# mlcolab/Pathfinder.jl

Measured on AMD Instinct MI355X. Metric: ELBO draws/sec (multipathfinder hot path: fit + ELBO + pool + PSIS + resample), higher is better.
Workload: dtype f64

## Files before the change

pathfinder.jl_amd/csrc/elbo_qf_kernel.hip:

```cpp
#include <type_traits>
#include <stdio.h>
#include <stdlib.h>
#include "pfmi_common.h"
#include "elbo_args.h"
#ifndef QF_PROF
#define QF_PROF 0
#endif

#ifndef QF_WAVES
#define QF_WAVES 8
#endif
#define QF_THREADS (QF_WAVES * 64)
#ifndef QF_NG
#define QF_NG 2
#endif
#ifndef QF_ABLATE
#define QF_ABLATE 0
#endif
#ifndef QF_PHILOX_HOIST
#define QF_PHILOX_HOIST 1
#endif
#ifndef QF_PSEUDO_FLIGHT
#define QF_PSEUDO_FLIGHT 1
#endif
#ifndef QF_CS_LDS
#define QF_CS_LDS 1
#endif
#ifndef QF_NG2_MAXKC
#define QF_NG2_MAXKC 20
#endif
#ifndef QF_PRIO_FAIR
#define QF_PRIO_FAIR 8
#endif
#ifndef QF_PRIO_YOUNG
#define QF_PRIO_YOUNG 0
#endif
#ifndef QF_SETPRIO
#define QF_SETPRIO 0
#endif
#define QF_MIN_FRONT 1024
static_assert(QF_MIN_FRONT >= 2 * PF_ICDF_BFE_FRONT, "the look-up's front guard");
template <int KC> struct qf_chb { static constexpr int v = (KC > 20) ? 8 : 16; };

#pragma clang fp contract(off)

typedef double qf_d4 __attribute__((ext_vector_type(4)));
__device__ __forceinline__ qf_d4 qf_mfma16(double a, double b, qf_d4 c) { return __builtin_amdgcn_mfma_f64_16x16x4f64(a, b, c, 0, 0, 0); }
__device__ __forceinline__ double qf_mfma4(double a, double b, double c) { return __builtin_amdgcn_mfma_f64_4x4x4f64(a, b, c, 0, 0, 0); }

__host__ __device__ constexpr int qf_nconst(int KC, int RPAD) { return 4 + KC + KC * KC + RPAD + RPAD * KC + KC; }

__host__ __device__ constexpr int qf_head_lds(int KC, int NG) { return (NG == 2 && KC < 16) ? 256 : 0; }

template <int TGT>
__device__ __forceinline__ void qf_row_ac(const ElboArgs &A, const double *mu, int i, double &a, double &c) {
    if (TGT == 1) { a = A.t_a[i]; c = mu[i] - A.t_mean[i]; }
    else if (TGT == 2) { a = (i >= 1) ? 1.0 : 0.0; c = mu[i]; }
    else { a = 0.0; c = 0.0; }
}

template <int KC>
__device__ __forceinline__ int qf_vh_pos(int lrow, int col) {
    const int bl = lrow >> 4, rr = lrow & 15, q = rr >> 2, r = rr & 3, T = col >> 2, i = col & 3;
    return (((bl * 4 + r) * (KC / 4) + T) << 4) + q * 4 + i;
}

struct QfKernArgs { ElboArgs A; int ch_blocks, nchunks, groups_per_wg, ngroups, n_whole, n_tail, ndep; double *cshare; unsigned *cflag; unsigned epoch; int cs_off; };
__host__ __device__ constexpr bool qf_cs_lds(int KC, int TGT, int NG) { return QF_CS_LDS != 0 && TGT != 0 && !(NG == 2 && KC >= 16); }
__device__ __forceinline__ int qf_arg_cs_off() {
    const char *ka = (const char *)__builtin_amdgcn_kernarg_segment_ptr();
    asm volatile("" : "+s"(ka));
    return *reinterpret_cast<const int *>(ka + offsetof(QfKernArgs, cs_off));
}
#ifndef QF_SHARE_SPINS
#define QF_SHARE_SPINS 2000000
#endif
template <int KC, int TGT, int RPAD, int NG>
__global__ __launch_bounds__(QF_THREADS) void pf_elbo_qf_kernel(ElboArgs A, int ch_blocks, int nchunks, int groups_per_wg, int ngroups, int n_whole,
                                                                  int n_tail, int ndep, double *, unsigned *, unsigned, int) {
    extern __shared__ __attribute__((aligned(16))) double lds[];
#if QF_PROF
    const long long qf_t0 = wall_clock64();
    long long qf_tb = 0, qf_te = 0, qf_tp = 0, qf_last = 0;
#endif
    constexpr int NT = KC / 4, TR = RPAD / 4, NC = qf_nconst(KC, RPAD);
    constexpr int QF_CHB = qf_chb<KC>::v;
    constexpr bool FOLD = !(NG == 2 && KC >= 16);
    constexpr bool PHX = QF_PHILOX_HOIST != 0;
    constexpr int PRE = (QF_CHB * 16 * KC + QF_THREADS - 1) / QF_THREADS;
    const int tid = threadIdx.x, wv = tid >> 6, lane = tid & 63, q = lane >> 4, c = lane & 15, l3 = lane & 3;
    const int d = A.d, nblk = (d + 15) >> 4;
    int slot = blockIdx.y, role = 0;
    int g_begin = blockIdx.x * groups_per_wg, g_cap = groups_per_wg;
    if (n_tail > 0 && slot >= n_whole) {
        constexpr int SL = QF_WAVES * NG, NPG_ = (TGT != 0) ? (KC + 1 + 15) / 16 : 0;
        int tail_f;
        if (slot < n_whole + n_tail) { role = 1; tail_f = slot - n_whole; g_begin = 0; g_cap = SL - NPG_; }
        else {
            const int t = slot - n_whole - n_tail;
            role = 2; tail_f = t / ndep;
            g_begin = (SL - NPG_) + (t - tail_f * ndep) * SL; g_cap = SL;
        }
        slot = n_whole + tail_f;
    }
    const int p = A.points[slot];
    const size_t blkidx = A.by_point ? (size_t)p : (size_t)slot;
    double *out_lp = A.logp + blkidx * A.log_stride, *out_lq = A.logq + blkidx * A.log_stride;
    constexpr int NPG = (TGT != 0) ? (KC + 1 + 15) / 16 : 0;
    const int npg = (role == 2) ? 0 : NPG;
    const int g_end = (g_begin + g_cap < ngroups) ? g_begin + g_cap : ngroups;
    const int nlb = (npg + (g_end - g_begin) + QF_WAVES * NG - 1) / (QF_WAVES * NG);
    if (A.status[p] != PFMI_FIT_OK) {
        for (int64_t n = (int64_t)g_begin * 16 + tid; n < (int64_t)g_end * 16 && n < A.N; n += QF_THREADS) {
            out_lp[n] = NAN; out_lq[n] = NAN;
        }
        return;
    }
    const int vh_sz = ch_blocks * 16 * KC, rs_sz = ch_blocks * 48;
    const int buf_stride = (nchunks > 1) ? vh_sz + rs_sz : 0;
    const int stage_sz = (nchunks > 1 ? 2 : 1) * (vh_sz + rs_sz);
    const int fix_off = stage_sz > QF_MIN_FRONT ? stage_sz : QF_MIN_FRONT;
    double *t_s = lds + fix_off;
    double *cn_s = t_s + KC * KC;
    double *g_s = cn_s + NC;
    double *h_s = g_s + RPAD * RPAD;
    double2 *icdf = reinterpret_cast<double2 *>(h_s + qf_head_lds(KC, NG) + ((KC * KC + NC + RPAD * RPAD) & 1));

    const double *Vh = A.vh + (size_t)p * d * KC, *mu = A.mu + (size_t)p * d, *sqa = A.sqrt_alpha + (size_t)p * d;
    auto stage_direct = [&](int ck, int buf) {
        const int row0 = ck * ch_blocks * 16;
        double *vs = lds + buf * buf_stride, *rs = vs + vh_sz;
        const int npair = ch_blocks * 8 * KC;
        const int lim = (d - row0) * KC;
        const double2 *src = reinterpret_cast<const double2 *>(Vh + (size_t)row0 * KC);
        constexpr int U = 6;
        for (int j0 = tid; j0 < npair; j0 += QF_THREADS * U) {
            double2 v[U];
#pragma unroll
            for (int u = 0; u < U; ++u) {
                const int j = j0 + u * QF_THREADS, jc = (2 * j + 1 < lim) ? j : (lim >> 1) - 1;
                v[u] = src[jc];
            }
#pragma unroll
            for (int u = 0; u < U; ++u) {
                const int j = j0 + u * QF_THREADS, idx = 2 * j;
                if (j < npair) {
                    const int lrow = idx / KC, col = idx - lrow * KC;
                    const double2 val = (idx < lim) ? v[u] : make_double2(0.0, 0.0);
                    *reinterpret_cast<double2 *>(vs + qf_vh_pos<KC>(lrow, col)) = val;
                }
            }
        }
        int cs_o = 0;
        if constexpr (qf_cs_lds(KC, TGT, NG)) { if (npg > 0) cs_o = qf_arg_cs_off(); }
        for (int l0 = tid; l0 < ch_blocks * 16; l0 += QF_THREADS * 2) {
            double a[2], cc[2], s[2];
#pragma unroll
            for (int u = 0; u < 2; ++u) {
                const int lrow = l0 + u * QF_THREADS, row = row0 + lrow, rc = row < d ? row : d - 1;
                qf_row_ac<TGT>(A, mu, rc, a[u], cc[u]);
                s[u] = sqa[rc];
            }
#pragma unroll
            for (int u = 0; u < 2; ++u) {
                const int lrow = l0 + u * QF_THREADS, row = row0 + lrow;
                if (lrow < ch_blocks * 16) {
                    const bool in = row < d;
                    double *o = rs + (lrow >> 4) * 48 + (lrow & 15);
                    o[0] = in ? a[u] * s[u] * s[u] : 0.0; o[16] = in ? 2.0 * a[u] * cc[u] * s[u] : 0.0; o[32] = in ? s[u] : 0.0;
                    if constexpr (qf_cs_lds(KC, TGT, NG)) { if (cs_o) lds[cs_o + lrow] = in ? cc[u] / s[u] : 0.0; }
                }
            }
        }
    };
    {
        const double *T = A.tmat + (size_t)p * KC * KC;
        for (int i = tid; i < KC * KC; i += QF_THREADS) t_s[i] = T[i];
        for (int i = tid; i < NC; i += QF_THREADS) cn_s[i] = 0.0;
        if (RPAD > 0) for (int i = tid; i < RPAD * RPAD; i += QF_THREADS) g_s[i] = A.t_g[i];
        pf_icdf_load(icdf);
        stage_direct(0, 0);
    }
    const int rho = 4 * (c & 3) + (c >> 2);
    constexpr bool HLDS = qf_head_lds(KC, NG) > 0;
    constexpr bool HREG = !(NG == 2 && KC >= 16) && !HLDS;
    const double *Vc = A.vchol + (size_t)p * KC * KC;
    auto head_op = [&](const int which, const int r) -> double {
        const int b = 4 * q + r;
        if (which == 0) { double v = (rho == b) ? 1.0 : 0.0; if (rho < KC && b < KC) v = Vc[b * KC + rho]; return v; }
        const int i1 = 16 + rho, b1 = 16 + b;
        if (which == 1) return (i1 < KC) ? Vc[b * KC + i1] : 0.0;
        double v1 = (i1 == b1) ? 1.0 : 0.0;
        if (i1 < KC && b1 < KC) v1 = Vc[b1 * KC + i1];
        return v1;
    };
    double a_h00[HREG ? 4 : 1], a_h10[HREG ? 4 : 1], a_h11[HREG ? 4 : 1];
    if (HREG) {
#pragma unroll
        for (int r = 0; r < 4; ++r) {
            a_h00[HREG ? r : 0] = head_op(0, r);
            a_h10[HREG ? r : 0] = (KC > 16) ? head_op(1, r) : 0.0;
            a_h11[HREG ? r : 0] = (KC > 16) ? head_op(2, r) : 0.0;
        }
    }
    if (HLDS && wv == 0) {
#pragma unroll
        for (int r = 0; r < 4; ++r) h_s[r * 64 + lane] = head_op(0, r);
    }
    auto hop = [&](const int which, const int r) -> double {
        if (HLDS) return h_s[r * 64 + lane];
        if (HREG) return which == 0 ? a_h00[HREG ? r : 0] : (which == 1 ? a_h10[HREG ? r : 0] : a_h11[HREG ? r : 0]);
        return head_op(which, r);
    };
    const uint64_t seed = A.seeds[slot];
    const uint32_t k0 = (uint32_t)seed, k1 = (uint32_t)(seed >> 32);
    const double logdet = A.logdet[p];
    __syncthreads();
#if QF_PROF
    qf_tp = wall_clock64() - qf_t0; qf_last = wall_clock64();
#endif
#if QF_PRIO_YOUNG
    if (wv >= 4) __builtin_amdgcn_s_setprio(1);
#endif
    if (TGT == 2) {
        if (tid == 0) { cn_s[1] = mu[0]; cn_s[2] = sqa[0]; }
        if (tid < KC) cn_s[4 + KC + KC * KC + RPAD + RPAD * KC + tid] = Vh[tid];
    }

    int cur = 0;
    for (int lb = 0; lb < nlb; ++lb) {
        bool pseudo[NG], active[NG];
        int sl[NG];
        int grp[NG];
        pf_philox_inv pinv[NG];
        auto draw_of = [&](const int g) -> uint32_t { return (uint32_t)(A.n0 + ((int64_t)grp[g] * 16 + c)); };
        double accw[NG][NT], acc3[NG][NT], acc4[NG][TR > 0 ? TR : 1];
        double usq[NG], q12[NG], z00[NG], u0[NG][4];
        bool any_active = false, any_pseudo = false, any_real = false;
#pragma unroll
        for (int g = 0; g < NG; ++g) {
            sl[g] = (lb * QF_WAVES + wv) * NG + g;
            pseudo[g] = sl[g] < npg;
            grp[g] = g_begin + sl[g] - npg;
            active[g] = pseudo[g] || grp[g] < g_end;
            if (PHX) {
                pinv[g] = pf_philox_draw_invariants(draw_of(g), k0, k1);
                if constexpr (NG == 2 && KC >= 16) asm volatile("" : "+v"(pinv[g].C), "+v"(pinv[g].D), "+v"(pinv[g].E), "+v"(pinv[g].F));
            }
            any_active |= active[g]; any_pseudo |= pseudo[g]; any_real |= active[g] && !pseudo[g];
#pragma unroll
            for (int T = 0; T < NT; ++T) { accw[g][T] = 0.0; acc3[g][T] = 0.0; }
#pragma unroll
            for (int T = 0; T < (TR > 0 ? TR : 1); ++T) acc4[g][T] = 0.0;
            usq[g] = 0.0; q12[g] = 0.0; z00[g] = 0.0;
#pragma unroll
            for (int r = 0; r < 4; ++r) u0[g][r] = 0.0;
        }
        struct Pend { uint32_t x[4]; double dp[4]; double2 c01[4], c23[4]; };
        const uint32_t icdf_adj = pf_icdf_adj_bfe<PF_ICDF_NB_LDS>(icdf);
        auto gen_issue = [&](const int g, const int blk, const uint64_t t, Pend &P) {
            auto words = [&](uint32_t (&x)[4]) {
                if (PHX) pf_philox4x32_hoisted<PF_NORMAL_ROUNDS>(pinv[g], t, k0, k1, x);
                else pf_philox_normals(draw_of(g), (uint32_t)(blk * 4 + q), 0u, 0u, k0, k1, x);
            };
#if QF_ABLATE == 1
#pragma unroll
            for (int r = 0; r < 4; ++r) { P.x[r] = 0x40000000u | (draw_of(g) + blk); P.dp[r] = 1e-3 * (blk + r); P.c01[r] = make_double2(0.1, 0.2); P.c23[r] = make_double2(0.3, 0.4); }
#elif QF_ABLATE == 2
            words(P.x);
#pragma unroll
            for (int r = 0; r < 4; ++r) { P.dp[r] = (double)P.x[r] * 0x1p-32; P.c01[r] = make_double2(0.1, 0.2); P.c23[r] = make_double2(0.3, 0.4); }
#else
            words(P.x);
#pragma unroll
            for (int r = 0; r < 4; ++r) pf_icdf_issue_bfe<PF_ICDF_NB_LDS>(P.x[r], icdf_adj, P.dp[r], P.c01[r], P.c23[r]);
#endif
        };
        for (int ck = 0; ck < nchunks; ++ck) {
            double pre[PRE], pr_s = 0.0, pr_a = 0.0, pr_c = 0.0;
            const int nck = (ck + 1 < nchunks) ? ck + 1 : 0;
            const bool do_pre = (nchunks > 1) && (ck + 1 < nchunks || lb + 1 < nlb);
            if (do_pre) {
                const int row0 = nck * QF_CHB * 16;
                int tid_p = tid;
                asm volatile("" : "+v"(tid_p));
#pragma unroll
                for (int e = 0; e < PRE; ++e) {
                    const int idx = tid_p + e * QF_THREADS;
                    const int lrow = idx / KC, row = row0 + lrow;
                    pre[e] = (idx < QF_CHB * 16 * KC && row < d) ? Vh[(size_t)row0 * KC + idx] : 0.0;
                }
                if (tid_p < QF_CHB * 16) {
                    const int row = row0 + tid_p;
                    if (row < d) { qf_row_ac<TGT>(A, mu, row, pr_a, pr_c); pr_s = sqa[row]; }
                }
            }
            if (any_active) {
                const double *vs = lds + cur * buf_stride, *rs = vs + vh_sz;
                const int blk0 = ck * ch_blocks;
                const int nb = (nblk - blk0 < ch_blocks) ? nblk - blk0 : ch_blocks;
                struct Ops { double av[4][NT]; double wd[4][TR > 0 ? TR : 1]; double rs[12]; };
                auto load_ops = [&](const int bl, Ops &o) {
                    const double *rp = rs + bl * 48 + 4 * q;
                    const double *ap = vs + ((bl * 4) * NT << 4) + q * 4 + l3;
#pragma unroll
                    for (int r = 0; r < 4; ++r) {
#pragma unroll
                        for (int T = 0; T < NT; ++T) o.av[r][T] = ap[(r * NT + T) << 4];
                        o.rs[r] = rp[r]; o.rs[4 + r] = rp[16 + r]; o.rs[8 + r] = rp[32 + r];
                    }
                    if (TGT == 1 && RPAD > 0) {
                        const double *wp = A.t_wd16 + ((size_t)(blk0 + bl) * 16 + 4 * q) * 16 + l3;
#pragma unroll
                        for (int r = 0; r < 4; ++r)
#pragma unroll
                            for (int T = 0; T < TR; ++T) o.wd[r][T] = wp[r * 16 + 4 * T];
                    }
                };
                auto contract = [&](const int g, const double (&z)[4], const Ops &o, const bool with_w) {
#if QF_SETPRIO
                    __builtin_amdgcn_s_setprio(QF_SETPRIO);
#endif
                    double bp[4], bs[4];
#pragma unroll
                    for (int r = 0; r < 4; ++r) {
                        bp[r] = 0.0; bs[r] = 0.0;
                        if (TGT != 0) bp[r] = (with_w && FOLD) ? fma(o.rs[r], z[r], o.rs[4 + r]) : o.rs[r] * z[r];
                        if (TGT == 1 && RPAD > 0) bs[r] = o.rs[8 + r] * z[r];
                    }
                    __builtin_amdgcn_sched_barrier(0);
#pragma unroll
                    for (int r = 0; r < 4; ++r) {
                        if (TGT != 0) q12[g] = fma((with_w && FOLD) ? bp[r] : bp[r] + o.rs[4 + r], z[r], q12[g]);
#pragma unroll
                        for (int T = 0; T < NT; ++T) {
                            if (with_w) accw[g][T] = qf_mfma4(o.av[r][T], z[r], accw[g][T]);
                            if (TGT != 0) acc3[g][T] = qf_mfma4(o.av[r][T], bp[r], acc3[g][T]);
                        }
                        if (TGT == 1 && RPAD > 0) {
#pragma unroll
                            for (int T = 0; T < TR; ++T) acc4[g][T] = qf_mfma4(o.wd[r][T], bs[r], acc4[g][T]);
                        }
                    }
#if QF_SETPRIO
                    __builtin_amdgcn_s_setprio(0);
#endif
                };
                auto normals = [&](const int g, const int blk, double (&z)[4]) {
                    uint32_t x[4];
                    pf_philox_normals(draw_of(g), (uint32_t)(blk * 4 + q), 0u, 0u, k0, k1, x);
                    pf_icdf4(x, draw_of(g), (uint32_t)(blk * 4 + q), 0u, k0, k1, icdf, z);
                    if (blk == nblk - 1) {
#pragma unroll
                        for (int r = 0; r < 4; ++r) z[r] = (blk * 16 + 4 * q + r < d) ? z[r] : 0.0;
                    }
#pragma unroll
                    for (int r = 0; r < 4; ++r) usq[g] = fma(z[r], z[r], usq[g]);
                    if (blk == 0) {
                        qf_d4 h = {0.0, 0.0, 0.0, 0.0};
#pragma unroll
                        for (int r = 0; r < 4; ++r) { u0[g][r] = z[r]; h = qf_mfma16(hop(0, r), z[r], h); }
#pragma unroll
                        for (int r = 0; r < 4; ++r) z[r] = h[r];
                        z00[g] = z[0];
                    } else if (KC > 16 && blk == 1) {
                        qf_d4 h = {0.0, 0.0, 0.0, 0.0};
#pragma unroll
                        for (int r = 0; r < 4; ++r) h = qf_mfma16(hop(1, r), u0[g][r], h);
#pragma unroll
                        for (int r = 0; r < 4; ++r) h = qf_mfma16(hop(2, r), z[r], h);
#pragma unroll
                        for (int r = 0; r < 4; ++r) z[r] = h[r];
                    }
                };
                auto finish = [&](const int g, const int blk, const Pend &P, double (&z)[4], auto special_tag) {
                    constexpr bool SPECIAL = decltype(special_tag)::value;
#pragma unroll
                    for (int r = 0; r < 4; ++r) z[r] = pf_icdf_finish(P.x[r], P.dp[r], P.c01[r], P.c23[r]);
                    if (__builtin_expect(__any(pf_icdf_miss4(P.x)), 0))
                        pf_icdf4_fix(P.x, draw_of(g), (uint32_t)(blk * 4 + q), 0u, k0, k1, z);
                    if (SPECIAL) {
                        if (blk == nblk - 1) {
#pragma unroll
                            for (int r = 0; r < 4; ++r) z[r] = (blk * 16 + 4 * q + r < d) ? z[r] : 0.0;
                        }
#pragma unroll
                        for (int r = 0; r < 4; ++r) usq[g] = fma(z[r], z[r], usq[g]);
                        if (blk == 0) {
                            qf_d4 h = {0.0, 0.0, 0.0, 0.0};
#pragma unroll
                            for (int r = 0; r < 4; ++r) { u0[g][r] = z[r]; h = qf_mfma16(hop(0, r), z[r], h); }
#pragma unroll
                            for (int r = 0; r < 4; ++r) z[r] = h[r];
                            z00[g] = z[0];
                        } else if (KC > 16 && blk == 1) {
                            qf_d4 h = {0.0, 0.0, 0.0, 0.0};
#pragma unroll
                            for (int r = 0; r < 4; ++r) h = qf_mfma16(hop(1, r), u0[g][r], h);
#pragma unroll
                            for (int r = 0; r < 4; ++r) h = qf_mfma16(hop(2, r), z[r], h);
#pragma unroll
                            for (int r = 0; r < 4; ++r) z[r] = h[r];
                        }
                    } else {
#pragma unroll
                        for (int r = 0; r < 4; ++r) usq[g] = fma(z[r], z[r], usq[g]);
                    }
                };
                auto pseudo_cols = [&](const int g, const int blk, const int bl, const int cs_o, double (&z)[4]) {
                    const int j = 16 * sl[g] + c;
                    if (qf_cs_lds(KC, TGT, NG) && cs_o != 0) {
                        const double *cs = lds + cs_o + bl * 16 + 4 * q;
#pragma unroll
                        for (int r = 0; r < 4; ++r) {
                            double v = 0.0;
                            if (j < KC) v = vs[qf_vh_pos<KC>(bl * 16 + 4 * q + r, j)];
                            else if (j == KC) v = cs[r];
                            z[r] = v;
                        }
                    } else if constexpr (QF_PSEUDO_FLIGHT != 0 && TGT == 1) {
                        double pm[4], ptm[4], ps[4];
#pragma unroll
                        for (int r = 0; r < 4; ++r) {
                            const int row = blk * 16 + 4 * q + r, rc = row < d ? row : d - 1;
                            pm[r] = mu[rc]; ptm[r] = A.t_mean[rc]; ps[r] = sqa[rc];
                        }
                        asm volatile("" ::: "memory");
                        __builtin_amdgcn_sched_barrier(0);
#pragma unroll
                        for (int r = 0; r < 4; ++r) {
                            const int row = blk * 16 + 4 * q + r;
                            double v = 0.0;
                            if (j < KC) v = vs[qf_vh_pos<KC>(bl * 16 + 4 * q + r, j)];
                            else if (j == KC && row < d) v = (pm[r] - ptm[r]) / ps[r];
                            z[r] = v;
                        }
                    } else {
#pragma unroll
                        for (int r = 0; r < 4; ++r) {
                            const int row = blk * 16 + 4 * q + r;
                            double v = 0.0;
                            if (j < KC) v = vs[qf_vh_pos<KC>(bl * 16 + 4 * q + r, j)];
                            else if (j == KC && row < d) {
                                double aa, cc;
                                qf_row_ac<TGT>(A, mu, row, aa, cc);
                                v = cc / sqa[row];
                            }
                            z[r] = v;
                        }
                    }
                };
                if (any_pseudo) {
                    int cs_o = 0;
                    if constexpr (qf_cs_lds(KC, TGT, NG)) cs_o = qf_arg_cs_off();
                    for (int bl = 0; bl < nb; ++bl) {
                        Ops oa;
                        load_ops(bl, oa);
#pragma unroll
                        for (int g = 0; g < NG; ++g) {
                            if (!active[g]) continue;
                            double z[4];
                            if (pseudo[g]) { pseudo_cols(g, blk0 + bl, bl, cs_o, z); contract(g, z, oa, false); }
                            else { normals(g, blk0 + bl, z); contract(g, z, oa, true); }
                        }
                    }
                } else {
                    auto block_body_seq = [&](const int bl, auto special_tag) {
                        const int blk = blk0 + bl;
                        double z[NG][4];
                        const uint64_t t = pf_philox_block_product((uint32_t)(blk * 4 + q), k0);
#pragma unroll
                        for (int g = 0; g < NG; ++g) {
                            Pend pp;
                            gen_issue(g, blk, t, pp);
                            finish(g, blk, pp, z[g], special_tag);
                        }
                        const double *rp = rs + bl * 48 + 4 * q;
                        const double *ap = vs + ((bl * 4) * NT << 4) + q * 4 + l3;
#pragma unroll
                        for (int r = 0; r < 4; ++r) {
                            double av[NT];
#pragma unroll
                            for (int T = 0; T < NT; ++T) av[T] = ap[(r * NT + T) << 4];
                            const double r0 = rp[r], r1 = rp[16 + r];
#pragma unroll
                            for (int g = 0; g < NG; ++g) {
                                const double zr = z[g][r];
                                double bp = 0.0;
                                if (TGT != 0) {
                                    bp = r0 * zr;
                                    q12[g] = fma(bp + r1, zr, q12[g]);
                                }
#pragma unroll
                                for (int T = 0; T < NT; ++T) {
                                    accw[g][T] = qf_mfma4(av[T], zr, accw[g][T]);
                                    if (TGT != 0) acc3[g][T] = qf_mfma4(av[T], bp, acc3[g][T]);
                                }
                            }
                            if (TGT == 1 && RPAD > 0) {
                                const double *wp = A.t_wd16 + ((size_t)(blk0 + bl) * 16 + 4 * q + r) * 16 + l3;
                                double wd[TR > 0 ? TR : 1];
#pragma unroll
                                for (int T = 0; T < TR; ++T) wd[T] = wp[4 * T];
                                const double r2 = rp[32 + r];
#pragma unroll
                                for (int g = 0; g < NG; ++g) {
                                    const double bs = r2 * z[g][r];
#pragma unroll
                                    for (int T = 0; T < TR; ++T) acc4[g][T] = qf_mfma4(wd[T], bs, acc4[g][T]);
                                }
                            }
                        }
                    };
                    auto block_body = [&](const int bl, auto special_tag) {
                        if constexpr (NG == 2 && KC >= 16) { block_body_seq(bl, special_tag); return; }
                        const int blk = blk0 + bl;
                        Ops oa;
                        load_ops(bl, oa);
                        __builtin_amdgcn_sched_barrier(0);
                        Pend pp[NG];
                        double z[NG][4];
                        const uint64_t t = pf_philox_block_product((uint32_t)(blk * 4 + q), k0);
#pragma unroll
                        for (int g = 0; g < NG; ++g) gen_issue(g, blk, t, pp[g]);
#pragma unroll
                        for (int g = 0; g < NG; ++g) {
                            finish(g, blk, pp[g], z[g], special_tag);
#if QF_ABLATE == 3
                            q12[g] += z[g][0] + z[g][1] + z[g][2] + z[g][3] + oa.av[0][0] + oa.rs[0];
#else
                            contract(g, z[g], oa, true);
#endif
                        }
                    };
                    __builtin_amdgcn_s_waitcnt(0xC07F);
                    auto prio_turn = [&](const int blk) {
#if QF_PRIO_FAIR
                        if ((blk & (QF_PRIO_FAIR - 1)) == 0) {
                            if (((blk / QF_PRIO_FAIR) ^ (wv >> 2) ^ lb) & 1) __builtin_amdgcn_s_setprio(1); else __builtin_amdgcn_s_setprio(0);
                        }
#endif
                    };
                    if constexpr (NG == 2 && KC >= 16) {
                        for (int bl = 0; bl < nb; ++bl) {
                            const int blk = blk0 + bl;
                            prio_turn(blk);
                            if (__builtin_expect((blk == 0) | (blk == nblk - 1) | (KC > 16 && blk == 1), 0)) block_body(bl, std::true_type{});
                            else block_body(bl, std::false_type{});
                        }
                    } else {
                        constexpr int LEAD = (KC > 16) ? 2 : 1;
                        const int s_lo = (LEAD - blk0 <= 0) ? 0 : (LEAD - blk0 < nb ? LEAD - blk0 : nb);
                        const int s_hi = (blk0 + nb == nblk) ? (nb - 1 > s_lo ? nb - 1 : s_lo) : nb;
#pragma unroll
                        for (int bl = 0; bl < LEAD; ++bl)
                            if (bl < s_lo) { prio_turn(blk0 + bl); block_body(bl, std::true_type{}); }
                        for (int bl = s_lo; bl < s_hi; ++bl) { prio_turn(blk0 + bl); block_body(bl, std::false_type{}); }
                        if (s_hi < nb) { prio_turn(blk0 + s_hi); block_body(s_hi, std::true_type{}); }
                    }
                }
            }
            if (nchunks > 1) {
                if (do_pre) {
                    double *vs = lds + (cur ^ 1) * buf_stride, *rs = vs + vh_sz;
                    int tid_e = tid;
                    asm volatile("" : "+v"(tid_e));
#pragma unroll
                    for (int e = 0; e < PRE; ++e) {
                        const int idx = tid_e + e * QF_THREADS;
                        if (idx < QF_CHB * 16 * KC) { const int lrow = idx / KC; vs[qf_vh_pos<KC>(lrow, idx - lrow * KC)] = pre[e]; }
                    }
                    if (tid_e < QF_CHB * 16) {
                        double *o = rs + (tid_e >> 4) * 48 + (tid_e & 15);
                        o[0] = pr_a * pr_s * pr_s; o[16] = 2.0 * pr_a * pr_c * pr_s; o[32] = pr_s;
                    }
                }
                __syncthreads();
                cur ^= 1;
            }
        }
#if QF_PROF
        { const long long t_ = wall_clock64(); qf_tb += t_ - qf_last; qf_last = t_; }
#endif
        if (NPG > 0 && lb == 0) {
            int lane_p = lane;
            asm volatile("" : "+v"(lane_p));
            const int qp = lane_p >> 4, cp = lane_p & 15;
#pragma unroll
            for (int g = 0; g < NG; ++g) {
                if (!pseudo[g]) continue;
                const int j = 16 * sl[g] + cp;
                double *vv = cn_s + 4, *Mm = cn_s + 4 + KC, *t0 = Mm + KC * KC, *Nn = t0 + RPAD;
                const double q4 = pf_sum_q(q12[g]);
#pragma unroll
                for (int T = 0; T < NT; ++T) {
                    const int a = 4 * T + qp;
                    if (j < KC) Mm[a * KC + j] = acc3[g][T];
                    else if (j == KC) vv[a] = acc3[g][T];
                }
#pragma unroll
                for (int T = 0; T < TR; ++T) {
                    const int jr = 4 * T + qp;
                    if (j < KC) Nn[jr * KC + j] = acc4[g][T];
                    else if (j == KC) t0[jr] = acc4[g][T];
                }
                if (j == KC && qp == 0) cn_s[0] = q4 / 3.0;
            }
            double *cshare = nullptr; unsigned *cflag = nullptr; unsigned epoch = 0u; int tail_f = 0, n_tail_l = 0;
            if (role != 0) {
                const char *ka = (const char *)__builtin_amdgcn_kernarg_segment_ptr();
                asm volatile("" : "+s"(ka));
                cshare = *reinterpret_cast<double *const *>(ka + offsetof(QfKernArgs, cshare));
                cflag = *reinterpret_cast<unsigned *const *>(ka + offsetof(QfKernArgs, cflag));
                epoch = *reinterpret_cast<const unsigned *>(ka + offsetof(QfKernArgs, epoch));
                n_tail_l = *reinterpret_cast<const int *>(ka + offsetof(QfKernArgs, n_tail));
                const int n_whole_l = *reinterpret_cast<const int *>(ka + offsetof(QfKernArgs, n_whole));
                tail_f = slot - n_whole_l;
            }
            if (role == 2) {
                if (tid == 0) {
                    int spins = 0;
                    while (__hip_atomic_load(cflag + tail_f, __ATOMIC_ACQUIRE, __HIP_MEMORY_SCOPE_AGENT) != epoch && spins < QF_SHARE_SPINS) {
                        __builtin_amdgcn_s_sleep(32); ++spins;
                    }
                    if (spins >= QF_SHARE_SPINS) { cn_s[3] = NAN; atomicAdd(cflag + n_tail_l, 1u); }
                }
                __syncthreads();
                const bool lost = cn_s[3] != 0.0;
                int tid_s = tid;
                asm volatile("" : "+v"(tid_s));
                const double *src = cshare + (size_t)tail_f * NC;
                double cv[(NC + QF_THREADS - 1) / QF_THREADS];
#pragma unroll
                for (int u = 0; u < (NC + QF_THREADS - 1) / QF_THREADS; ++u) {
                    const int i = tid_s + u * QF_THREADS;
                    cv[u] = __hip_atomic_load(src + (i < NC ? i : NC - 1), __ATOMIC_RELAXED, __HIP_MEMORY_SCOPE_AGENT);
                }
                __syncthreads();
#pragma unroll
                for (int u = 0; u < (NC + QF_THREADS - 1) / QF_THREADS; ++u) {
                    const int i = tid_s + u * QF_THREADS;
                    if (i < NC) cn_s[i] = lost ? NAN : cv[u];
                }
            }
            __syncthreads();
            if (role == 1) {
                double *dst = cshare + (size_t)tail_f * NC;
                for (int i = tid; i < NC; i += QF_THREADS) __hip_atomic_store(dst + i, cn_s[i], __ATOMIC_RELAXED, __HIP_MEMORY_SCOPE_AGENT);
                __threadfence();
                __syncthreads();
                if (tid == 0) __hip_atomic_store(cflag + tail_f, epoch, __ATOMIC_RELEASE, __HIP_MEMORY_SCOPE_AGENT);
            }
        }
        if (!any_real) continue;
        int lane_e = lane;
        asm volatile("" : "+v"(lane_e));
        const int qe = lane_e >> 4, ce = lane_e & 15;
        int wv_e = tid;
        asm volatile("" : "+v"(wv_e));
        wv_e >>= 6;
        int d_e = d;
        asm volatile("" : "+s"(d_e));
#pragma unroll
        for (int g = 0; g < NG; ++g) {
            if (!active[g] || pseudo[g]) continue;
            double us = usq[g];
            us = pf_sum_q(us);
            double lp = NAN;
            if (TGT != 0) {
                double qs = q12[g];
                qs = pf_sum_q(qs);
                auto matvec = [&](const double *Mat, const int ld, const int nrows, auto nx_tag, auto ny_tag, auto lower_tag,
                                  const double (&x)[decltype(nx_tag)::value], double (&y)[decltype(ny_tag)::value]) {
                    constexpr int NX = decltype(nx_tag)::value, NY = decltype(ny_tag)::value;
                    constexpr bool LOWER = decltype(lower_tag)::value;
#pragma unroll
                    for (int rt = 0; rt < (NY + 3) / 4; ++rt) {
                        qf_d4 acc = {0.0, 0.0, 0.0, 0.0};
                        const int row = 16 * rt + ce;
#pragma unroll
                        for (int st = 0; st < NX; ++st) {
                            const int col = 4 * st + qe;
                            const bool ok = row < nrows && (!LOWER || col <= row);
                            const double av = ok ? Mat[row * ld + col] : 0.0;
                            acc = qf_mfma16(av, x[st], acc);
                        }
#pragma unroll
                        for (int r = 0; r < 4; ++r) if (4 * rt + r < NY) y[4 * rt + r] = acc[r];
                    }
                };
                const double *vv = cn_s + 4, *Mm = cn_s + 4 + KC, *t0 = Mm + KC * KC, *Nn = t0 + RPAD, *vh0 = Nn + RPAD * KC;
                double tvd[NT], mt[NT];
                matvec(t_s, KC, KC, std::integral_constant<int, NT>{}, std::integral_constant<int, NT>{}, std::false_type{}, accw[g], tvd);
                matvec(Mm, KC, KC, std::integral_constant<int, NT>{}, std::integral_constant<int, NT>{}, std::false_type{}, tvd, mt);
                double qa = 0.0;
#pragma unroll
                for (int T = 0; T < NT; ++T)
                    qa = fma(tvd[T], mt[T] - 2.0 * (FOLD ? acc3[g][T] - vv[4 * T + qe] : vv[4 * T + qe] + acc3[g][T]), qa);
                qa = pf_sum_q(qa);
                const double q1 = cn_s[0] + qs + qa;
                if (TGT == 1) {
                    double corr = 0.0;
                    if (RPAD > 0) {
                        constexpr int TRr = TR > 0 ? TR : 1;
                        double nt[TRr], tt[TRr], gg[TRr];
                        matvec(Nn, KC, RPAD, std::integral_constant<int, NT>{}, std::integral_constant<int, TRr>{}, std::false_type{}, tvd, nt);
#pragma unroll
                        for (int T = 0; T < TR; ++T) tt[T] = t0[4 * T + qe] + acc4[g][T] - nt[T];
                        matvec(g_s, RPAD, RPAD, std::integral_constant<int, TRr>{}, std::integral_constant<int, TRr>{}, std::true_type{}, tt, gg);
#pragma unroll
                        for (int T = 0; T < TR; ++T) corr = fma(gg[T], gg[T], corr);
                        corr = pf_sum_q(corr);
                    }
                    lp = A.t_offset - 0.5 * (q1 - corr);
                } else {
                    const double zh = __shfl(z00[g], ce, 64);
                    double pr = 0.0;
#pragma unroll
                    for (int T = 0; T < NT; ++T) pr = fma(vh0[4 * T + qe], tvd[T], pr);
                    pr = pf_sum_q(pr);
                    const double ta = cn_s[1] + cn_s[2] * (zh - pr), t3 = ta / 3.0;
                    lp = (t3 * t3 + (double)(d_e - 1) * ta + q1 * exp(-ta)) / -2.0;
                }
            }
            const int64_t nl = (int64_t)(g_begin + (lb * QF_WAVES + wv_e) * NG + g - npg) * 16 + ce;
            if (qe == 0 && nl < A.N) {
                out_lq[nl] = ((double)d_e * PF_LOG2PI + logdet + us) / -2.0;
                out_lp[nl] = lp;
            }
        }
#if QF_PROF
        { const long long t_ = wall_clock64(); qf_te += t_ - qf_last; qf_last = t_; }
#endif
    }
#if QF_PROF
    if (g_begin == 0 && (slot & 1023) == 3 && lane == 0)
        printf("QF_PROF fit %d wave %d (10 ns ticks): prologue %lld blocks %lld epilogue+publish %lld total %lld batches %d\n", slot, wv, qf_tp, qf_tb,
               qf_te, (long long)(wall_clock64() - qf_t0), nlb);
#endif
}

static size_t qf_lds_bytes(int ch_blocks, int nchunks, int kc, int rpad, int ng) {
    const size_t per = (size_t)ch_blocks * 16 * kc + (size_t)ch_blocks * 48;
    size_t stage = per * (nchunks > 1 ? 2 : 1);
    if (stage < QF_MIN_FRONT) stage = QF_MIN_FRONT;
    return sizeof(double) * (stage + (size_t)kc * kc + qf_nconst(kc, rpad) + (size_t)rpad * rpad + qf_head_lds(kc, ng) + 1 + 4 * PF_ICDF_LDS_ENTRIES + 2 * PF_ICDF_BFE_BEHIND);
}

static void qf_note_plan(pfmi_ctx *c, int kc, int tgt, int rpad, int ng, bool streamed, const char *cut) {
    char nm[64];
    snprintf(nm, sizeof nm, "qf:%d,%d,%d,%d:%s:%s", kc, tgt, rpad, ng, streamed ? "stream" : "res", cut);
    ++c->qf_plans[nm];
}

template <int KC, int TGT, int RPAD, int NG>
static int32_t launch_qf_ng(pfmi_ctx *c, const ElboArgs &a, int64_t nfits) {
    const int nblk = (a.d + 15) / 16;
    int ch_blocks = nblk, nchunks = 1;
    constexpr int QF_CHB = qf_chb<KC>::v;
    if (qf_lds_bytes(nblk, 1, KC, RPAD, NG) > 156 * 1024) { ch_blocks = QF_CHB; nchunks = (nblk + QF_CHB - 1) / QF_CHB; }
    size_t lds_bytes = qf_lds_bytes(ch_blocks, nchunks, KC, RPAD, NG);
    int cs_off = 0;
    const char *no_cs = pf_debug_get("PFMI_QF_NO_CS_LDS");
    if (qf_cs_lds(KC, TGT, NG) && nchunks == 1 && !(no_cs && no_cs[0] == '1') &&
        lds_bytes + sizeof(double) * 16 * (size_t)ch_blocks <= 160 * 1024) {
        cs_off = (int)(lds_bytes / sizeof(double));
        lds_bytes += sizeof(double) * 16 * (size_t)ch_blocks;
    }
    PF_CHECK(lds_bytes <= 160 * 1024, PFMI_ERR_UNSUPPORTED, "qf kernel LDS %zu too large", lds_bytes);
    auto kern = pf_elbo_qf_kernel<KC, TGT, RPAD, NG>;
    PF_TRY(pf_raise_lds_limit(c, reinterpret_cast<const void *>(kern), 160 * 1024));
    const int ngroups = (int)((a.N + 15) / 16);
    constexpr int NPG = (TGT != 0) ? (KC + 1 + 15) / 16 : 0;
    int split = 1;
    while (!c->qf_seg_mode && (int64_t)split * nfits < 1024 && (ngroups + NPG) / (split * 2) >= QF_WAVES * NG) split *= 2;
    int gpw = (ngroups + split - 1) / split;
    if (split > 1) gpw = ((gpw + NPG + QF_WAVES * NG - 1) / (QF_WAVES * NG)) * (QF_WAVES * NG) - NPG;
    if (gpw < 1) gpw = 1;
    const int gx = (ngroups + gpw - 1) / gpw;
    auto launch = [&](int64_t f0, int64_t nf, int gpw_, int gx_) {
        for (int64_t s0 = f0; s0 < f0 + nf; s0 += 32768) {
            const int64_t ns = (f0 + nf - s0 < 32768) ? (f0 + nf - s0) : 32768;
            ElboArgs b = a;
            b.points = a.points + s0; b.seeds = a.seeds + s0;
            if (!a.by_point) { b.logp += s0 * a.log_stride; b.logq += s0 * a.log_stride; }
            hipLaunchKernelGGL(kern, dim3((unsigned)gx_, (unsigned)ns), dim3(QF_THREADS), lds_bytes, c->stream, b, ch_blocks, nchunks, gpw_,
                               ngroups, 0, 0, 0, (double *)nullptr, (unsigned *)nullptr, 0u, cs_off);
        }
    };
    int64_t tail = 0;
    int gpw_t = gpw, gx_t = gx, ndep = 0;
    const char *no_tail = pf_debug_get("PFMI_QF_NO_TAIL");
    const char *two = pf_debug_get("PFMI_QF_TWO_LAUNCHES");
    const bool two_launches = (two && two[0] == '1') || c->qf_no_share;
    if (split == 1 && TGT != 0 && !(no_tail && no_tail[0] == '1') && !c->qf_seg_mode) {
        int ncu = 0;
        PF_HIP(hipDeviceGetAttribute(&ncu, hipDeviceAttributeMultiprocessorCount, c->device));
        if (c->ncu_eff > 0 && c->ncu_eff < ncu) ncu = c->ncu_eff;
        const int slots = QF_WAVES * NG, nb_full = (ngroups + NPG + slots - 1) / slots;
        const int64_t rem = ncu > 0 ? nfits % ncu : 0;
        gpw_t = slots - NPG;
        gx_t = gpw_t > 0 ? (ngroups + gpw_t - 1) / gpw_t : 0;
        ndep = (ngroups > gpw_t) ? (ngroups - gpw_t + slots - 1) / slots : 0;
        const bool share_ok = !two_launches && gpw_t > 0 && (nfits - rem) + rem * (1 + ndep) <= 65535;
        const int pieces = share_ok ? 1 + ndep : gx_t;
        if (rem > 0 && nfits > ncu && gpw_t > 0 && nb_full > 1 && (rem * pieces + ncu - 1) / ncu < nb_full) tail = rem;
        if (tail > 0 && share_ok) {
            constexpr int NC = qf_nconst(KC, RPAD);
            const size_t cbytes = (size_t)tail * NC * sizeof(double), fbytes = ((size_t)tail + 1) * sizeof(unsigned);
            DevBuf &share = c->qf_share_s[c->qf_slot];
            uint32_t &epoch = c->qf_epoch_s[c->qf_slot];
            if (share.cap < cbytes + fbytes || epoch == 0xFFFFFFFFu) {
                PF_CHECK(!c->stream_pending, PFMI_ERR_STATE, "scan: the hand-over buffer of a streaming call must be allocated before its first launch");
                PF_TRY(share.ensure(cbytes + fbytes + (64 << 10)));
                PF_HIP(hipMemsetAsync(share.p, 0, share.cap, c->stream));
                epoch = 0;
            }
            unsigned *cflag = reinterpret_cast<unsigned *>(share.as<char>() + share.cap) - (tail + 1);
            hipLaunchKernelGGL(kern, dim3(1, (unsigned)((nfits - tail) + tail * (1 + ndep))), dim3(QF_THREADS), lds_bytes, c->stream, a, ch_blocks,
                               nchunks, gpw, ngroups, (int)(nfits - tail), (int)tail, ndep, share.as<double>(), cflag, ++epoch, cs_off);
            qf_note_plan(c, KC, TGT, RPAD, NG, nchunks > 1, "tail-share");
            return PFMI_OK;
        }
    }
    if (nfits - tail > 0) launch(0, nfits - tail, gpw, gx);
    if (tail > 0) launch(nfits - tail, tail, gpw_t, gx_t);
    qf_note_plan(c, KC, TGT, RPAD, NG, nchunks > 1, tail > 0 ? "tail-two" : (split > 1 ? "split" : "whole"));
    return PFMI_OK;
}

template <int KC, int TGT, int RPAD>
static int32_t launch_qf(pfmi_ctx *c, const ElboArgs &a, int64_t nfits) {
    if constexpr (KC <= QF_NG2_MAXKC && QF_NG == 2) {
        if (a.N >= 768 && (KC <= 12 || nfits >= 128)) return launch_qf_ng<KC, TGT, RPAD, 2>(c, a, nfits);
    }
    return launch_qf_ng<KC, TGT, RPAD, 1>(c, a, nfits);
}

template <int KC>
static int32_t launch_qf_t(pfmi_ctx *c, const ElboArgs &a, int64_t nfits, int tgt, int rpad) {
    if (tgt == 0) return launch_qf<KC, 0, 0>(c, a, nfits);
    if (tgt == 2) return launch_qf<KC, 2, 0>(c, a, nfits);
    if (rpad == 0) return launch_qf<KC, 1, 0>(c, a, nfits);
    if (rpad == 8) return launch_qf<KC, 1, 8>(c, a, nfits);
    return launch_qf<KC, 1, 16>(c, a, nfits);
}

int32_t pf_launch_elbo_qf(pfmi_ctx *c, const ElboArgs &a, int64_t nfits, int tgt, int rpad, bool *handled) {
    *handled = false;
    if (a.u != nullptr || a.x != nullptr) return PFMI_OK;
    int32_t rc = PFMI_OK;
    *handled = pf_dispatch_kpad<4, 8, 12, 16, 20, 32>(c->kpad, [&](auto KP) { rc = launch_qf_t<KP()>(c, a, nfits, tgt, rpad); });
    return rc;
}
```

Before: 528.7 million.

## Batch epilogue matvecs across draw groups and use 4x4 MFMA for small KC

Restructures the per-batch epilogue so the matrix operands (T, M, N, G) are loaded into registers once and the matvecs for all NG draw groups run interleaved, instead of reloading and computing per group. For KC<=12 it switches to 4x4 MFMA tiles rather than 16x16 so less padded work is done. The aim is to cut redundant LDS loads and expose independent MFMA chains. In exchange it raises register pressure, which could reduce occupancy or cause spills, and the pseudo/inactive groups are now computed and only skipped at the store.

Result: faster. 536.0 million (median of 6 runs) (+1.4%).

```diff
diff --git a/pathfinder.jl_amd/csrc/elbo_qf_kernel.hip b/pathfinder.jl_amd/csrc/elbo_qf_kernel.hip
--- a/pathfinder.jl_amd/csrc/elbo_qf_kernel.hip
+++ b/pathfinder.jl_amd/csrc/elbo_qf_kernel.hip
@@ -25,6 +25,12 @@
 #endif
 #ifndef QF_CS_LDS
 #define QF_CS_LDS 1
+#endif
+#ifndef QF_EPI_PAIR
+#define QF_EPI_PAIR 1
+#endif
+#ifndef QF_EPI_MFMA4
+#define QF_EPI_MFMA4 1
 #endif
 #ifndef QF_NG2_MAXKC
 #define QF_NG2_MAXKC 20
@@ -661,6 +667,147 @@
         wv_e >>= 6;
         int d_e = d;
         asm volatile("" : "+s"(d_e));
+#if QF_EPI_PAIR
+        {
+            constexpr bool M4 = QF_EPI_MFMA4 != 0 && KC <= 12;
+            constexpr int TRr = TR > 0 ? TR : 1;
+            constexpr int NRT = M4 ? NT : (NT + 3) / 4, NRR = M4 ? TRr : (TRr + 3) / 4;
+            constexpr bool LOWR = TGT == 1 && RPAD > 0;
+            using acc_t = std::conditional_t<M4, double, qf_d4>;
+            const int l3e = lane_e & 3;
+            auto load_a = [&](const double *Mat, const int ld, const int nrows, auto lower_tag, auto &a) {
+                constexpr bool LOWER = decltype(lower_tag)::value;
+                constexpr int NR = sizeof(a) / sizeof(a[0]), NX = sizeof(a[0]) / sizeof(double);
+#pragma unroll
+                for (int rt = 0; rt < NR; ++rt) {
+                    const int row = M4 ? 4 * rt + l3e : 16 * rt + ce;
+#pragma unroll
+                    for (int st = 0; st < NX; ++st) {
+                        const int col = 4 * st + qe;
+                        const bool ok = row < nrows && (!LOWER || col <= row);
+                        a[rt][st] = ok ? Mat[row * ld + col] : 0.0;
+                    }
+                }
+            };
+            auto mv_step = [&](const int st, const auto &a, const auto &x, auto &acc) {
+                constexpr int NR = sizeof(a) / sizeof(a[0]);
+#pragma unroll
+                for (int rt = 0; rt < NR; ++rt)
+#pragma unroll
+                    for (int g = 0; g < NG; ++g) {
+                        if constexpr (M4) acc[g][rt] = qf_mfma4(a[rt][st], x[g][st], acc[g][rt]);
+                        else acc[g][rt] = qf_mfma16(a[rt][st], x[g][st], acc[g][rt]);
+                    }
+            };
+            auto mv_zero = [&](auto &acc) {
+                constexpr int NR = sizeof(acc[0]) / sizeof(acc_t);
+#pragma unroll
+                for (int g = 0; g < NG; ++g)
+#pragma unroll
+                    for (int rt = 0; rt < NR; ++rt) acc[g][rt] = acc_t{};
+            };
+            auto mv_out = [&](const auto &acc, auto &y) {
+                constexpr int NR = sizeof(acc[0]) / sizeof(acc_t), NY = sizeof(y[0]) / sizeof(double);
+#pragma unroll
+                for (int g = 0; g < NG; ++g)
+#pragma unroll
+                    for (int rt = 0; rt < NR; ++rt) {
+                        if constexpr (M4) { if (rt < NY) y[g][rt] = acc[g][rt]; }
+                        else {
+#pragma unroll
+                            for (int r = 0; r < 4; ++r) if (4 * rt + r < NY) y[g][4 * rt + r] = acc[g][rt][r];
+                        }
+                    }
+            };
+            const double *vv = cn_s + 4, *Mm = cn_s + 4 + KC, *t0 = Mm + KC * KC, *Nn = t0 + RPAD, *vh0 = Nn + RPAD * KC;
+            double aT[NRT][NT], aM[NRT][NT], aN[NRR][NT], aG[NRR][TRr];
+            if (TGT != 0) {
+                load_a(t_s, KC, KC, std::false_type{}, aT);
+                load_a(Mm, KC, KC, std::false_type{}, aM);
+                if (LOWR) {
+                    load_a(Nn, KC, RPAD, std::false_type{}, aN);
+                    load_a(g_s, RPAD, RPAD, std::true_type{}, aG);
+                }
+                __builtin_amdgcn_sched_barrier(0);
+            }
+            double us[NG], lp[NG];
+#pragma unroll
+            for (int g = 0; g < NG; ++g) { us[g] = pf_sum_q(usq[g]); lp[g] = NAN; }
+            if (TGT != 0) {
+                double qs[NG], tvd[NG][NT], mt[NG][NT], nt[NG][TRr], q1[NG];
+                acc_t cT[NG][NRT], cM[NG][NRT], cN[NG][NRR];
+#pragma unroll
+                for (int g = 0; g < NG; ++g) qs[g] = pf_sum_q(q12[g]);
+                mv_zero(cT);
+#pragma unroll
+                for (int st = 0; st < NT; ++st) mv_step(st, aT, accw, cT);
+                mv_out(cT, tvd);
+                mv_zero(cM);
+                if (LOWR) mv_zero(cN);
+#pragma unroll
+                for (int st = 0; st < NT; ++st) {
+                    mv_step(st, aM, tvd, cM);
+                    if (LOWR) mv_step(st, aN, tvd, cN);
+                }
+                mv_out(cM, mt);
+                if (LOWR) mv_out(cN, nt);
+#pragma unroll
+                for (int g = 0; g < NG; ++g) {
+                    double qa = 0.0;
+#pragma unroll
+                    for (int T = 0; T < NT; ++T)
+                        qa = fma(tvd[g][T], mt[g][T] - 2.0 * (FOLD ? acc3[g][T] - vv[4 * T + qe] : vv[4 * T + qe] + acc3[g][T]), qa);
+                    qa = pf_sum_q(qa);
+                    q1[g] = cn_s[0] + qs[g] + qa;
+                }
+                if (TGT == 1) {
+                    double corr[NG];
+#pragma unroll
+                    for (int g = 0; g < NG; ++g) corr[g] = 0.0;
+                    if (RPAD > 0) {
+                        double tt[NG][TRr], gg[NG][TRr];
+                        acc_t cG[NG][NRR];
+#pragma unroll
+                        for (int g = 0; g < NG; ++g)
+#pragma unroll
+                            for (int T = 0; T < TR; ++T) tt[g][T] = t0[4 * T + qe] + acc4[g][T] - nt[g][T];
+                        mv_zero(cG);
+#pragma unroll
+                        for (int st = 0; st < TRr; ++st) mv_step(st, aG, tt, cG);
+                        mv_out(cG, gg);
+#pragma unroll
+                        for (int g = 0; g < NG; ++g) {
+#pragma unroll
+                            for (int T = 0; T < TR; ++T) corr[g] = fma(gg[g][T], gg[g][T], corr[g]);
+                            corr[g] = pf_sum_q(corr[g]);
+                        }
+                    }
+#pragma unroll
+                    for (int g = 0; g < NG; ++g) lp[g] = A.t_offset - 0.5 * (q1[g] - corr[g]);
+                } else {
+#pragma unroll
+                    for (int g = 0; g < NG; ++g) {
+                        const double zh = __shfl(z00[g], ce, 64);
+                        double pr = 0.0;
+#pragma unroll
+                        for (int T = 0; T < NT; ++T) pr = fma(vh0[4 * T + qe], tvd[g][T], pr);
+                        pr = pf_sum_q(pr);
+                        const double ta = cn_s[1] + cn_s[2] * (zh - pr), t3 = ta / 3.0;
+                        lp[g] = (t3 * t3 + (double)(d_e - 1) * ta + q1[g] * exp(-ta)) / -2.0;
+                    }
+                }
+            }
+#pragma unroll
+            for (int g = 0; g < NG; ++g) {
+                if (!active[g] || pseudo[g]) continue;
+                const int64_t nl = (int64_t)(g_begin + (lb * QF_WAVES + wv_e) * NG + g - npg) * 16 + ce;
+                if (qe == 0 && nl < A.N) {
+                    out_lq[nl] = ((double)d_e * PF_LOG2PI + logdet + us[g]) / -2.0;
+                    out_lp[nl] = lp[g];
+                }
+            }
+        }
+#else
 #pragma unroll
         for (int g = 0; g < NG; ++g) {
             if (!active[g] || pseudo[g]) continue;
@@ -729,6 +876,7 @@
                 out_lp[nl] = lp;
             }
         }
+#endif
 #if QF_PROF
         { const long long t_ = wall_clock64(); qf_te += t_ - qf_last; qf_last = t_; }
 #endif
```
